# qutech/filter_functions

Hardware: AMD Instinct MI355X
Metric: filter-function elements/sec (n_seg*n_omega*n_nops*d^2) at d=4 (higher is better)
Workload: dtype f64

## Files before the change

### filter_functions_amd/csrc/ctrl_pq.hip

```cpp
#include <algorithm>
#include <cstdlib>

#include "ffk_internal.h"
#include "ffk_mfma_util.h"

namespace ffk {
namespace {

constexpr int kPqProducers = 4;
constexpr int kPqSets = 2;
constexpr int kPqConsumers = 16/kPqSets;
constexpr int kPqRing = 8;
#ifndef FFK_PC_SPIN_LIMIT
#define FFK_PC_SPIN_LIMIT (1 << 21)
#endif
constexpr int kPqSpinLimit = FFK_PC_SPIN_LIMIT;

__device__ __forceinline__ void pq_report_fault(int* fault, int code) {
    if (fault != nullptr && (threadIdx.x & 63) == 0)
        __hip_atomic_store(fault, code, __ATOMIC_RELAXED, __HIP_MEMORY_SCOPE_SYSTEM);
}

typedef double double2_t __attribute__((ext_vector_type(2)));
typedef double double4_t __attribute__((ext_vector_type(4)));
typedef double double8_t __attribute__((ext_vector_type(8)));
typedef int int4_t __attribute__((ext_vector_type(4)));
typedef __attribute__((address_space(3))) int lds_int_t;

template <int NC>
struct PqConsumer;
#include "ctrl_pq_consumer.inc"

constexpr int kPqQ = 0, kPqPsi = 1024, kPqW = 1152;
constexpr int kPqRow = seg_stride(4);
__host__ __device__ constexpr int pq_tile_doubles(int nc) { return kPqW + nc*128 + 32; }
__host__ __device__ constexpr int pq_lds_bytes_for(int nc) {
    return (kPqRing*pq_tile_doubles(nc) + kPqProducers*kPqRow)*8 + 3*kPqRing*4;
}

__device__ __forceinline__ int lds_peek(const int* flag) {
    return __builtin_amdgcn_readfirstlane(*(const volatile lds_int_t*)(flag));
}

template <int NC, bool PRE>
__global__ __launch_bounds__((kPqProducers + kPqConsumers)*64, 3) void ctrl_accumulate_pq_kernel(
    const double* __restrict__ omega, int W, const double* __restrict__ segtab,
    const cplx* __restrict__ ops, int G, int A, int chunk_len, cplx* __restrict__ Ypart,
    const cplx* __restrict__ wfold, int alpha_base, int alpha_end, int* __restrict__ fault_word) {
    constexpr int D = 4, DD = 16, S = kPqRow, TILE = pq_tile_doubles(NC);
    constexpr int TOP = kPqW + NC*128;
    static_assert(PqConsumer<NC>::kTileBytes == TILE*8, "tools/gen_pq_consumer.py and pq_tile_doubles() disagree");
    extern __shared__ __attribute__((aligned(16))) unsigned char lds_raw[];
    double* ring = reinterpret_cast<double*>(lds_raw);
    double* rows = ring + kPqRing*TILE;
    int* ready = reinterpret_cast<int*>(rows + kPqProducers*S);
    int* done = ready + kPqRing;

    const int lane = threadIdx.x & 63;
    const int wave = __builtin_amdgcn_readfirstlane(threadIdx.x >> 6);
    const int alpha0 = alpha_base + blockIdx.y*NC;
    const int n_alpha = min(NC, alpha_end - alpha0);
    const int g0 = blockIdx.z*chunk_len;
    const int g1 = min(G, g0 + chunk_len);
    const int n_it = max(0, g1 - g0);
    int spin_limit = kPqSpinLimit;

    if (threadIdx.x < 3*kPqRing) *(volatile lds_int_t*)(ready + threadIdx.x) = 0;
    __syncthreads();

    if (wave < kPqProducers) {
        __builtin_amdgcn_s_setprio(0);
        const int iw = blockIdx.x*64 + lane;
        double om = omega[iw < W ? iw : W - 1];
        asm volatile("" : "+v"(om));
        const int n_ops = (1 + n_alpha)*DD;
        double* row = rows + wave*S;
        struct Staged {
            cplx o;
            double r0, r1;
        };
        auto request = [&](int it) __attribute__((always_inline)) -> Staged {
            const int g = g0 + it;
            const cplx* src = ops + static_cast<size_t>(g)*(1 + A)*DD;
            const double* st = segtab + static_cast<size_t>(g)*S;
            Staged t;
            if constexpr (PRE) {
                t.o = cplx{0.0, 0.0};
                t.r0 = st[lane];
                t.r1 = st[64 + (lane & (S - 64 - 1))];
            } else {
                t.o = lane < n_ops ? src[lane < DD ? lane : lane + alpha0*DD] : cplx{0.0, 0.0};
                t.r0 = st[lane];
                t.r1 = lane < S - 64 ? st[64 + lane] : 0.0;
            }
            return t;
        };
        auto wait_slot = [&](int slot, int gen) __attribute__((always_inline)) {
            if (gen > 0) {
                int spin = 0;
                for (; spin < spin_limit; ++spin) {
                    if (lds_peek(done + slot) >= gen*kPqConsumers) break;
                    __builtin_amdgcn_s_sleep(2);
                }
                if (spin == spin_limit && spin_limit != 0) {
                    pq_report_fault(fault_word, kFaultPcProducerWait);
                    spin_limit = 0;
                }
                asm volatile("" ::: "memory");
            }
        };
        Staged cur = {};
        if (wave < n_it) cur = request(wave);
        for (int it = wave; it < n_it; it += kPqProducers) {
            const int slot = it & (kPqRing - 1);
            const int gen = it/kPqRing;
            double* buf = ring + slot*TILE;
            row[lane] = cur.r0;
            if (lane < S - 64) row[64 + lane] = cur.r1;
            const cplx o = cur.o;
            if constexpr (PRE) {
                wait_slot(slot, gen);
                const size_t gw = (static_cast<size_t>(g0 + it)*A + alpha0)*64;
#pragma unroll
                for (int a = 0; a < NC; ++a)
                    if (a < n_alpha) lds_dma16(wfold + gw + a*64 + lane, buf + kPqW + a*128);
                if (lane < DD) lds_dma16(ops + static_cast<size_t>(g0 + it)*(1 + A)*DD + lane, buf + TOP);
            }
            if (it + kPqProducers < n_it) cur = request(it + kPqProducers);
            const double* st = row;
            const double2_t sbcb = *reinterpret_cast<const double2_t*>(st + seg_rec(lane >> 2) + 1);
            const double2_t head = *reinterpret_cast<const double2_t*>(st);
            const double sb = sbcb.x, cb = sbcb.y;
            const double dtg = head.x;
            cplx ph;
            sincos_pi<false>(om*head.y, &ph.im, &ph.re);
            double sa, ca;
            sincos_pi<false>(0.5*(om*dtg), &sa, &ca);
            const PhasedFrequency pf = phased_frequency(om, dtg, ph, sa, ca);
            double q[DD];
            auto batch = [&](int e0, int e1) __attribute__((always_inline)) {
                double4_t rec[DD];
#pragma unroll
                for (int e = 0; e < DD; ++e) {
                    if (e < e0 || e >= e1 || (e != 0 && e/D == e%D)) continue;
                    rec[e] = *reinterpret_cast<const double4_t*>(st + seg_rec(e));
                }
                asm volatile("" ::: "memory");
                double xmin = pf.thr;
#pragma unroll
                for (int e = 0; e < DD; ++e) {
                    if (e < e0 || e >= e1 || (e != 0 && e/D == e%D)) continue;
                    const double x = om + rec[e].x;
                    q[e] = fma(pf.sa2, rec[e].z, pf.ca2*rec[e].y)*rcp_fast(x);
                    asm("v_min_f64 %0, |%1|, %0" : "+v"(xmin) : "v"(x));
                }
                if (xmin < pf.thr) {
#pragma unroll
                    for (int e = 0; e < DD; ++e) {
                        if (e < e0 || e >= e1 || (e != 0 && e/D == e%D)) continue;
                        if (fabs(om + rec[e].x) < pf.thr) q[e] = phased_q(pf, rec[e].x, rec[e].y, rec[e].z);
                    }
                }
            };
            batch(0, 8);
            batch(8, 16);
            q[5] = q[0];
            q[10] = q[0];
            q[15] = q[0];
            if constexpr (!PRE) wait_slot(slot, gen);
#pragma unroll
            for (int h = 0; h < 2; ++h)
#pragma unroll
                for (int m = 0; m < D; ++m) {
                    const double2_t v = {q[m*D + 2*h], q[m*D + 2*h + 1]};
                    *reinterpret_cast<double2_t*>(buf + kPqQ + h*512 + lane*8 + (((m ^ (lane >> 2)) & 3) << 1)) = v;
                }
            {
                const double2_t v = {pf.pr, pf.pi};
                *reinterpret_cast<double2_t*>(buf + kPqPsi + lane*2) = v;
            }
            if constexpr (!PRE) {
                const int src_t = lane & (DD - 1);
                const cplx tv = {__shfl(o.re, src_t, 64), __shfl(o.im, src_t, 64)};
                const cplx et = cmul(cplx{cb, sb}, tv);
                const int wslot = ((lane >> 2) & 3)*16 + (lane >> 4)*4 + (lane & 3);
#pragma unroll
                for (int a = 0; a < NC; ++a) {
                    const int src_b = DD + a*DD + (lane >> 2);
                    const cplx bv = {__shfl(o.re, src_b, 64), __shfl(o.im, src_b, 64)};
                    const cplx w = cmul(bv, et);
                    const double2_t v = {w.re, w.im};
                    *reinterpret_cast<double2_t*>(buf + kPqW + a*128 + wslot*2) = v;
                }
            }
            if constexpr (PRE) {
                if (it + kPqProducers < n_it) asm volatile("s_waitcnt vmcnt(2)" ::: "memory");
                else lds_dma_wait();
            } else if (lane < DD) {
                const double2_t v = {o.re, o.im};
                *reinterpret_cast<double2_t*>(buf + TOP + lane*2) = v;
            }
            asm volatile("s_waitcnt lgkmcnt(0)" ::: "memory");
#ifdef FFK_PC_FAULT_INJECT
            if (it < 2*kPqProducers)
#endif
            if (lane == 0) *(volatile lds_int_t*)(ready + slot) = it + 1;
        }
        return;
    }

    const int octant = wave - kPqProducers;
    const int m = lane >> 4, f = (lane >> 2) & 3, j = lane & 3;
    const int mj = m*4 + j;
    const int wf = octant*4*kPqSets + f;
    const int o_w = kPqW + mj*2;
    const int o_p = kPqPsi + wf*2;
    const int o_q0 = kPqQ + wf*8 + ((m ^ ((kPqSets*octant) & 3)) << 1);
    const int o_q1 = (o_q0 ^ 2) + 32;
    double P[6*NC];
#pragma unroll
    for (int k = 0; k < 6*NC; ++k) P[k] = 0.0;
    if (n_it > 0) {
        int spin = 0;
        for (; spin < spin_limit; ++spin) {
            if (lds_peek(ready) >= 1) break;
            __builtin_amdgcn_s_sleep(1);
        }
        if (spin == spin_limit) {
            pq_report_fault(fault_word, kFaultPcConsumerWait);
            spin_limit = 0;
        }
        asm volatile("" ::: "memory");
        const unsigned ring_b = static_cast<unsigned>(reinterpret_cast<uintptr_t>(ring));
        const unsigned flags_b = static_cast<unsigned>(reinterpret_cast<uintptr_t>(ready));
        const int fault_code = PqConsumer<NC>::run(ring_b + o_w*8, ring_b + o_q0*8, ring_b + o_q1*8, ring_b + o_p*8, n_it,
                                                   spin_limit, flags_b, octant, P);
        if (fault_code != 0) pq_report_fault(fault_word, fault_code);
    }
#pragma unroll
    for (int a = 0; a < NC; ++a) {
        const int alpha = alpha0 + a;
        if (alpha >= alpha_end) break;
        cplx* out = Ypart + ((static_cast<size_t>(blockIdx.z)*A + alpha)*DD + mj)*W;
#pragma unroll
        for (int s = 0; s < kPqSets; ++s) {
            const int iw = blockIdx.x*64 + wf + s*4;
            const double p1 = P[3*(kPqSets*a + s)], p2 = P[3*(kPqSets*a + s) + 1], p3 = P[3*(kPqSets*a + s) + 2];
            if (iw < W) out[iw] = cplx{p1 - p2, p3 - (p1 + p2)};
        }
    }
}

template <int NC, bool PRE>
hipError_t launch_pq_as(const double* omega, int W, const double* segtab, const cplx* ops, int G, int A,
                        int chunks, int chunk_len, cplx* Ypart, const cplx* wfold, int alpha_base, int alpha_end,
                        int* fault_word, hipStream_t stream) {
    const int lds = pq_lds_bytes_for(NC);
    auto kern = ctrl_accumulate_pq_kernel<NC, PRE>;
    hipError_t err = hipFuncSetAttribute(reinterpret_cast<const void*>(kern),
                                         hipFuncAttributeMaxDynamicSharedMemorySize, lds);
    if (err != hipSuccess) return err;
    const int n = alpha_end - alpha_base;
    const dim3 grid((W + 63)/64, (n + NC - 1)/NC, chunks);
    hipLaunchKernelGGL(kern, grid, dim3((kPqProducers + kPqConsumers)*64), lds, stream, omega, W, segtab,
                       ops, G, A, chunk_len, Ypart, wfold, alpha_base, alpha_end, fault_word);
    return hipGetLastError();
}

template <int NC>
hipError_t launch_pq(const double* omega, int W, const double* segtab, const cplx* ops, int G, int A,
                     int chunks, int chunk_len, cplx* Ypart, const cplx* wfold, int alpha_base, int alpha_end,
                     int* fault_word, hipStream_t stream) {
    return wfold != nullptr ? launch_pq_as<NC, true>(omega, W, segtab, ops, G, A, chunks, chunk_len, Ypart, wfold,
                                                     alpha_base, alpha_end, fault_word, stream)
                            : launch_pq_as<NC, false>(omega, W, segtab, ops, G, A, chunks, chunk_len, Ypart, nullptr,
                                                      alpha_base, alpha_end, fault_word, stream);
}

}

int pq_accumulate_lds_bytes(int nc) { return pq_lds_bytes_for(nc); }
int pq_accumulate_waves(int) { return kPqProducers + kPqConsumers; }
bool pq_accumulate_supported(int d, int A) { return d == 4 && A >= 1; }

PqGroups pq_accumulate_groups(int A) {
    if (A <= 0) return {0, 0, 0};
    if (A == 1) return {0, 0, 1};
    switch (A % 3) {
        case 0: return {A/3, 0, 0};
        case 1: return {(A - 4)/3, 2, 0};
        default: return {(A - 2)/3, 1, 0};
    }
}

hipError_t launch_accumulate_pq(const double* omega, int W, const double* segtab, const cplx* ops,
                                int G, int d, int A, int chunks, int chunk_len, cplx* Ypart,
                                const cplx* wfold, hipStream_t stream) {
    if (d != 4) return hipErrorInvalidValue;
    int* fault_word = kernel_fault_word();
    const PqGroups g = pq_accumulate_groups(A);
    hipError_t err = hipSuccess;
    int base = 0;
    if (g.n3 > 0) {
        err = launch_pq<3>(omega, W, segtab, ops, G, A, chunks, chunk_len, Ypart, wfold, base, base + 3*g.n3,
                           fault_word, stream);
        base += 3*g.n3;
    }
    if (err == hipSuccess && g.n2 > 0) {
        err = launch_pq<2>(omega, W, segtab, ops, G, A, chunks, chunk_len, Ypart, wfold, base, base + 2*g.n2,
                           fault_word, stream);
        base += 2*g.n2;
    }
    if (err == hipSuccess && g.n1 > 0)
        err = launch_pq<1>(omega, W, segtab, ops, G, A, chunks, chunk_len, Ypart, wfold, base, base + g.n1,
                           fault_word, stream);
    return err;
}

}
```

### filter_functions_amd/csrc/ffk_math.h

```cpp
#pragma once

#include <hip/hip_runtime.h>

#include <cmath>

#define FFK_HD __host__ __device__ __forceinline__

namespace ffk {

struct cplx {
    double re, im;
};

FFK_HD cplx cmul(cplx a, cplx b) {
    return {fma(a.re, b.re, -(a.im*b.im)), fma(a.re, b.im, a.im*b.re)};
}
FFK_HD void cmac(cplx& acc, cplx a, cplx b) {
    acc.re = fma(a.re, b.re, acc.re);
    acc.re = fma(-a.im, b.im, acc.re);
    acc.im = fma(a.re, b.im, acc.im);
    acc.im = fma(a.im, b.re, acc.im);
}
FFK_HD void cmac_conj(cplx& acc, cplx a, cplx b) {
    acc.re = fma(a.re, b.re, acc.re);
    acc.re = fma(a.im, b.im, acc.re);
    acc.im = fma(a.re, b.im, acc.im);
    acc.im = fma(-a.im, b.re, acc.im);
}

template <unsigned long long BITS>
FFK_HD double pinned_bits() {
#if defined(__HIP_DEVICE_COMPILE__)
    unsigned lo, hi;
    asm volatile("v_mov_b32 %0, %1" : "=v"(lo) : "n"(static_cast<unsigned>(BITS & 0xffffffffull)));
    asm volatile("v_mov_b32 %0, %1" : "=v"(hi) : "n"(static_cast<unsigned>(BITS >> 32)));
    return __hiloint2double(static_cast<int>(hi), static_cast<int>(lo));
#else
    return __builtin_bit_cast(double, BITS);
#endif
}
#define FFK_PIN(c) (PIN ? pinned_bits<__builtin_bit_cast(unsigned long long, static_cast<double>(c))>() : (c))

template <bool PIN = false>
FFK_HD void sincos_reduced(double r, double* s, double* c) {
    const double z = r*r;
    double ps = fma(z, FFK_PIN(1.58969099521155010221e-10), FFK_PIN(-2.50507602534068634195e-08));
    ps = fma(z, ps, FFK_PIN(2.75573137070700676789e-06));
    ps = fma(z, ps, FFK_PIN(-1.98412698298579493134e-04));
    ps = fma(z, ps, FFK_PIN(8.33333333332248946124e-03));
    ps = fma(z, ps, FFK_PIN(-1.66666666666666324348e-01));
    *s = fma(r*z, ps, r);
    double pc = fma(z, FFK_PIN(-1.13596475577881948265e-11), FFK_PIN(2.08757232129817482790e-09));
    pc = fma(z, pc, FFK_PIN(-2.75573143513906633035e-07));
    pc = fma(z, pc, FFK_PIN(2.48015872894767294178e-05));
    pc = fma(z, pc, FFK_PIN(-1.38888888888741095749e-03));
    pc = fma(z, pc, FFK_PIN(4.16666666666666019037e-02));
    const double hz = 0.5*z;
    const double w = 1.0 - hz;
    *c = w + (((1.0 - w) - hz) + z*z*pc);
}

template <bool PIN = false>
FFK_HD void sincos_small(double r, double* s, double* c) {
    const double z = r*r;
    double ps = fma(z, FFK_PIN(2.75573137070700676789e-06), FFK_PIN(-1.98412698298579493134e-04));
    ps = fma(z, ps, FFK_PIN(8.33333333332248946124e-03));
    ps = fma(z, ps, FFK_PIN(-1.66666666666666324348e-01));
    *s = fma(r*z, ps, r);
    double pc = fma(z, FFK_PIN(2.48015872894767294178e-05), FFK_PIN(-1.38888888888741095749e-03));
    pc = fma(z, pc, FFK_PIN(4.16666666666666019037e-02));
    const double hz = 0.5*z;
    const double w = 1.0 - hz;
    *c = w + (((1.0 - w) - hz) + z*z*pc);
}

FFK_HD unsigned low_word(double t) {
#if defined(__HIP_DEVICE_COMPILE__)
    return static_cast<unsigned>(__double2loint(t));
#else
    unsigned long long bits;
    __builtin_memcpy(&bits, &t, sizeof bits);
    return static_cast<unsigned>(bits);
#endif
}

template <bool PIN = false>
FFK_HD void sincos_pi(double x, double* s, double* c) {
    const double kMagic = FFK_PIN(6755399441055744.0);
    const double t = fma(x, FFK_PIN(6.36619772367581382433e-01), kMagic);
    const unsigned q = low_word(t);
    const double k = t - kMagic;
    double r = fma(-k, FFK_PIN(1.57079632679489655800e+00), x);
    r = fma(-k, FFK_PIN(6.12323399573676603587e-17), r);
    r = fma(-k, FFK_PIN(-1.49738490485916983294e-33), r);
    double sr, cr;
    sincos_reduced<PIN>(r, &sr, &cr);
    const double s0 = (q & 1u) ? cr : sr;
    const double c0 = (q & 1u) ? sr : cr;
    *s = (q & 2u) ? -s0 : s0;
    *c = ((q + 1u) & 2u) ? -c0 : c0;
}

#undef FFK_PIN

FFK_HD double rcp(double x) {
#if defined(__HIP_DEVICE_COMPILE__)
    double y = __builtin_amdgcn_rcp(x);
    double e = fma(-x, y, 1.0);
    y = fma(y, e, y);
    e = fma(-x, y, 1.0);
    y = fma(y, e, y);
    return y;
#else
    return 1.0/x;
#endif
}

FFK_HD double rcp_fast(double x) {
#if defined(__HIP_DEVICE_COMPILE__)
    double y = __builtin_amdgcn_rcp(x);
    const double e = fma(-x, y, 1.0);
    return fma(y, e, y);
#else
    return 1.0/x;
#endif
}

FFK_HD double rsqrt(double x) {
#if defined(__HIP_DEVICE_COMPILE__)
    double y = __builtin_amdgcn_rsq(x);
    double e = fma(-x*y, y, 1.0);
    y = fma(y, 0.5*e, y);
    e = fma(-x*y, y, 1.0);
    y = fma(y, 0.5*e, y);
    return y;
#else
    return 1.0/sqrt(x);
#endif
}

FFK_HD cplx first_order_integral(double omega, double dE, double dt) {
    const double x = omega + dE;
    const double y = x*dt;
    double s, c;
    sincos_pi(0.5*y, &s, &c);
    const double q = 2.0*s*rcp(x);
    cplx out = {q*c, q*s};
    if (x == 0.0) {
        out.re = dt;
        out.im = 0.0;
    }
    return out;
}

FFK_HD cplx first_order_integral_aa(double omega, double dE, double dt, double sa, double ca,
                                    double sb, double cb) {
    const double x = omega + dE;
    const double h = 0.5*(x*dt);
    double s = fma(sa, cb, ca*sb);
    double c = fma(ca, cb, -(sa*sb));
    if (fabs(h) < 0.03125) sincos_small<true>(h, &s, &c);
    const double q = 2.0*s*rcp_fast(x);
    cplx out = {q*c, q*s};
    if (x == 0.0) {
        out.re = dt;
        out.im = 0.0;
    }
    return out;
}

struct PhasedFrequency {
    double om, dt, thr;
    double pr, pi;
    double sa2, ca2;
};
FFK_HD PhasedFrequency phased_frequency(double om, double dt, cplx ph, double sa, double ca) {
    PhasedFrequency f;
    f.om = om;
    f.dt = dt;
    f.thr = dt > 0.0 ? 0.0625*rcp(dt) : __builtin_huge_val();
    f.pr = fma(ph.re, ca, -(ph.im*sa));
    f.pi = fma(ph.re, sa, ph.im*ca);
    f.sa2 = sa + sa;
    f.ca2 = ca + ca;
    return f;
}
FFK_HD double phased_q(const PhasedFrequency& f, double dE, double sb, double cb) {
    const double x = f.om + dE;
    double q;
    if (fabs(x) < f.thr) {
        double s, c;
        sincos_small<true>(0.5*(x*f.dt), &s, &c);
        q = x == 0.0 ? f.dt : 2.0*s*rcp_fast(x);
    } else {
        q = fma(f.sa2, cb, f.ca2*sb)*rcp_fast(x);
    }
    return q;
}
FFK_HD cplx phased_integral_aa(const PhasedFrequency& f, double dE, double sb, double cb) {
    const double er = fma(f.pr, cb, -(f.pi*sb));
    const double ei = fma(f.pr, sb, f.pi*cb);
    const double q = phased_q(f, dE, sb, cb);
    return {q*er, q*ei};
}

template <bool PIN = false>
FFK_HD cplx cexp(double x) {
    cplx out;
    sincos_pi<PIN>(x, &out.im, &out.re);
    return out;
}

constexpr double kDerivativeIntegralBand = 0.0009765625;
constexpr double kDerivativeIntegralTaylor = 0.001953125;

#define FFK_PINNED(c) pinned_bits<__builtin_bit_cast(unsigned long long, static_cast<double>(c))>()

template <int J>
FFK_HD void derivative_integral_series_step(double X, cplx& S) {
    const double f = X*FFK_PINNED(1.0/(J + 1));
    S = {fma(-f, S.im, FFK_PINNED(1.0/(J + 5))), f*S.re};
    if constexpr (J > 0) derivative_integral_series_step<J - 1>(X, S);
}

FFK_HD double derivative_integral_rcp(double b, double dt) {
    return fabs(b*dt) < kDerivativeIntegralBand ? 0.0 : 1.0/b;
}

FFK_HD cplx derivative_integral_sum(double B, double unit, cplx m1, cplx m2, cplx m3, cplx m4) {
    const double B4 = 0.25*B, B2 = 0.5*B;
    const double B3 = FFK_PINNED(1.0/3.0)*B;
    cplx h = {fma(-B4, m4.im, m3.re), fma(B4, m4.re, m3.im)};
    h = {fma(-B3, h.im, m2.re), fma(B3, h.re, m2.im)};
    h = {fma(-B2, h.im, m1.re), fma(B2, h.re, m1.im)};
    return {unit*h.re, unit*h.im};
}

FFK_HD cplx derivative_integral(double x, double b, double rb, double dt, cplx i1x, cplx i1xb) {
    const cplx df = {i1xb.re - i1x.re, i1xb.im - i1x.im};
    cplx j = {df.im*rb, -df.re*rb};
    const double X = x*dt;
    const double up = rb == 0.0 ? fabs(X) : -1.0, down = rb == 0.0 ? fabs(X) : 1.0;
    if (up >= kDerivativeIntegralTaylor) {
        const cplx ex = {1.0 - x*i1x.im, x*i1x.re};
        const double rx = 1.0/x;
        const cplx m1 = {(dt*ex.im - i1x.im)*rx, -(dt*ex.re - i1x.re)*rx};
        double p = dt*dt;
        const cplx m2 = {(p*ex.im - 2.0*m1.im)*rx, -(p*ex.re - 2.0*m1.re)*rx};
        p *= dt;
        const cplx m3 = {(p*ex.im - 3.0*m2.im)*rx, -(p*ex.re - 3.0*m2.re)*rx};
        p *= dt;
        const cplx m4 = {(p*ex.im - 4.0*m3.im)*rx, -(p*ex.re - 4.0*m3.re)*rx};
        j = derivative_integral_sum(b, 1.0, m1, m2, m3, m4);
    }
    if (down < kDerivativeIntegralTaylor) {
        const cplx ex = {1.0 - x*i1x.im, x*i1x.re};
        cplx m4 = {FFK_PINNED(1.0/10.0), 0.0};
        derivative_integral_series_step<4>(X, m4);
        const double third = FFK_PINNED(1.0/3.0);
        const cplx m3 = {0.25*(ex.re + X*m4.im), 0.25*(ex.im - X*m4.re)};
        const cplx m2 = {(ex.re + X*m3.im)*third, (ex.im - X*m3.re)*third};
        const cplx m1 = {0.5*(ex.re + X*m2.im), 0.5*(ex.im - X*m2.re)};
        j = derivative_integral_sum(b*dt, dt*dt, m1, m2, m3, m4);
    }
    return j;
}

struct SecondOrderMoments {
    cplx m1, m2, m3, m4;
};

FFK_HD SecondOrderMoments second_order_moments(double a, double dt, cplx i1a) {
    const double X = a*dt;
    const cplx ex = {1.0 - a*i1a.im, a*i1a.re};
    SecondOrderMoments m;
    if (fabs(X) >= kDerivativeIntegralTaylor) {
        const double rX = 1.0/X, rdt = 1.0/dt;
        m.m1 = {(ex.im - i1a.im*rdt)*rX, -(ex.re - i1a.re*rdt)*rX};
        m.m2 = {(ex.im - 2.0*m.m1.im)*rX, -(ex.re - 2.0*m.m1.re)*rX};
        m.m3 = {(ex.im - 3.0*m.m2.im)*rX, -(ex.re - 3.0*m.m2.re)*rX};
        m.m4 = {(ex.im - 4.0*m.m3.im)*rX, -(ex.re - 4.0*m.m3.re)*rX};
    } else {
        m.m4 = {0.1, 0.0};
        derivative_integral_series_step<4>(X, m.m4);
        m.m3 = {0.25*(ex.re + X*m.m4.im), 0.25*(ex.im - X*m.m4.re)};
        m.m2 = {(ex.re + X*m.m3.im)*(1.0/3.0), (ex.im - X*m.m3.re)*(1.0/3.0)};
        m.m1 = {0.5*(ex.re + X*m.m2.im), 0.5*(ex.im - X*m.m2.re)};
    }
    return m;
}

FFK_HD cplx second_order_series(double b, double dt, cplx s1, cplx s2, cplx s3, cplx s4) {
    return derivative_integral_sum(b*dt, dt*dt, s1, s2, s3, s4);
}

FFK_HD cplx second_order_integral(double a, double b, double ab, double dt) {
    const cplx i1a = first_order_integral(a, 0.0, dt);
    const double rb = derivative_integral_rcp(b, dt);
    if (rb == 0.0) {
        const SecondOrderMoments m = second_order_moments(a, dt, i1a);
        return second_order_series(b, dt, m.m1, m.m2, m.m3, m.m4);
    }
    const cplx i1ab = first_order_integral(ab, 0.0, dt);
    return {-(i1a.im - i1ab.im)*rb, (i1a.re - i1ab.re)*rb};
}

#undef FFK_PINNED

}
```

### filter_functions_amd/csrc/prep.hip

```cpp
#include "ffk_internal.h"

namespace ffk {
namespace {

template <int D>
__device__ void prologue_segment(const cplx (*V)[D], cplx (*Q)[D], cplx (*T)[D], cplx (*BV)[D],
                                 int g, int lane, const double* __restrict__ eigvals,
                                 const cplx* __restrict__ n_opers,
                                 const double* __restrict__ n_coeffs,
                                 const double* __restrict__ dt, const double* __restrict__ t, int G,
                                 int A, double* __restrict__ segtab, cplx* __restrict__ Tc,
                                 cplx* __restrict__ ops, cplx* __restrict__ n_opers_transformed,
                                 cplx* __restrict__ eigvecs_propagated, bool with_noise_ops = true,
                                 cplx* __restrict__ wfold = nullptr) {
    constexpr int S = seg_stride(D);
    double* st = segtab + static_cast<size_t>(g)*S;
    if (lane == 0) {
        st[0] = dt[g];
        st[1] = t[g];
    }
    cplx eb = {1.0, 0.0};
    for (int e = lane; e < D*D; e += 64) {
        const double dE = eigvals[static_cast<size_t>(g)*D + e / D] - eigvals[static_cast<size_t>(g)*D + e % D];
        double sb, cb;
        sincos_pi(0.5*(dE*dt[g]), &sb, &cb);
        st[seg_rec(e)] = dE;
        st[seg_rec(e) + 1] = sb;
        st[seg_rec(e) + 2] = cb;
        st[seg_rec(e) + 3] = 0.0;
        eb = {cb, sb};
    }
    if (lane < 2) st[2 + lane] = 0.0;
    for (int e = 4 + 4*D*D + lane; e < S; e += 64) st[e] = 0.0;

    for (int e = lane; e < D*D; e += 64) {
        const int m = e / D, j = e % D;
        cplx acc = {0.0, 0.0};
#pragma unroll
        for (int k = 0; k < D; ++k) cmac_conj(acc, V[k][m], Q[k][j]);
        T[m][j] = acc;
        Tc[static_cast<size_t>(g)*D*D + e] = {acc.re, -acc.im};
        ops[static_cast<size_t>(g)*(1 + A)*D*D + e] = acc;
        if (eigvecs_propagated)
            eigvecs_propagated[static_cast<size_t>(g)*D*D + j*D + m] = {acc.re, -acc.im};
    }
    __syncthreads();

    if (!with_noise_ops) return;
    const bool fold = D == 4 && wfold != nullptr;
    if (fold) {
        if (lane < D*D) Q[lane / D][lane % D] = eb;
        __syncthreads();
    }
    for (int a = 0; a < A; ++a) {
        const cplx* B = n_opers + static_cast<size_t>(a)*D*D;
        const double s = n_coeffs ? n_coeffs[static_cast<size_t>(a)*G + g] : 1.0;
        for (int e = lane; e < D*D; e += 64) {
            const int i = e / D, n = e % D;
            cplx acc = {0.0, 0.0};
#pragma unroll
            for (int k = 0; k < D; ++k) cmac(acc, B[i*D + k], V[k][n]);
            BV[i][n] = acc;
        }
        __syncthreads();
        cplx bbar = {0.0, 0.0};
        for (int e = lane; e < D*D; e += 64) {
            const int m = e / D, n = e % D;
            cplx acc = {0.0, 0.0};
#pragma unroll
            for (int k = 0; k < D; ++k) cmac_conj(acc, V[k][m], BV[k][n]);
            acc.re *= s;
            acc.im *= s;
            ops[(static_cast<size_t>(g)*(1 + A) + 1 + a)*D*D + e] = acc;
            if (n_opers_transformed)
                n_opers_transformed[(static_cast<size_t>(a)*G + g)*D*D + e] = acc;
            if (fold) bbar = acc;
        }
        __syncthreads();
        if (fold) {
            if (lane < D*D) BV[lane / D][lane % D] = bbar;
            __syncthreads();
            if constexpr (D == 4) {
                const int m = lane >> 4, n = (lane >> 2) & 3, j = lane & 3;
                const cplx et = cmul(Q[m][n], T[n][j]);
                const cplx w = cmul(BV[m][n], et);
                wfold[(static_cast<size_t>(g)*A + a)*64 + n*16 + m*4 + j] = w;
            }
            __syncthreads();
        }
    }
}

template <int D>
__global__ __launch_bounds__(64) void prologue_kernel(
    const double* __restrict__ eigvals, const cplx* __restrict__ eigvecs,
    const cplx* __restrict__ propagators, const cplx* __restrict__ n_opers,
    const double* __restrict__ n_coeffs, const double* __restrict__ dt,
    const double* __restrict__ t, int G, int A, double* __restrict__ segtab,
    cplx* __restrict__ Tc, cplx* __restrict__ ops, cplx* __restrict__ n_opers_transformed,
    cplx* __restrict__ eigvecs_propagated, bool with_noise_ops, cplx* __restrict__ wfold) {
    __shared__ cplx V[D][D];
    __shared__ cplx Q[D][D];
    __shared__ cplx T[D][D];
    __shared__ cplx BV[D][D];
    const int g = blockIdx.x;
    const int lane = threadIdx.x;
    for (int e = lane; e < D*D; e += 64) {
        V[e / D][e % D] = eigvecs[static_cast<size_t>(g)*D*D + e];
        Q[e / D][e % D] = propagators[static_cast<size_t>(g)*D*D + e];
    }
    __syncthreads();
    prologue_segment<D>(V, Q, T, BV, g, lane, eigvals, n_opers, n_coeffs, dt, t, G, A, segtab, Tc,
                        ops, n_opers_transformed, eigvecs_propagated, with_noise_ops, wfold);
}

template <int D>
__global__ __launch_bounds__(64) void prologue_pulses_kernel(
    const double* __restrict__ eigvals, const cplx* __restrict__ eigvecs,
    const cplx* __restrict__ propagators, const cplx* __restrict__ n_opers,
    const double* __restrict__ n_coeffs, const double* __restrict__ dt,
    const double* __restrict__ t, int G, int A, double* __restrict__ segtab,
    cplx* __restrict__ Tc, cplx* __restrict__ ops, cplx* __restrict__ n_opers_transformed) {
    __shared__ cplx V[D][D];
    __shared__ cplx Q[D][D];
    __shared__ cplx T[D][D];
    __shared__ cplx BV[D][D];
    constexpr size_t DD = D*D;
    const size_t p = blockIdx.y;
    const int g = blockIdx.x;
    const int lane = threadIdx.x;
    const cplx* Vp = eigvecs + p*G*DD;
    const cplx* Qp = propagators + p*(G + 1)*DD;
    for (int e = lane; e < D*D; e += 64) {
        V[e / D][e % D] = Vp[static_cast<size_t>(g)*DD + e];
        Q[e / D][e % D] = Qp[static_cast<size_t>(g)*DD + e];
    }
    __syncthreads();
    prologue_segment<D>(V, Q, T, BV, g, lane, eigvals + p*G*D, n_opers + p*A*DD, n_coeffs + p*A*G, dt + p*G,
                        t + p*(G + 1), G, A, segtab + p*G*seg_stride(D), Tc + p*G*DD, ops + p*G*(1 + A)*DD,
                        n_opers_transformed + p*A*G*DD, nullptr, true, nullptr);
}

template <int D>
__global__ __launch_bounds__(64) void noise_ops_kernel(const cplx* __restrict__ eigvecs,
                                                       const cplx* __restrict__ n_opers,
                                                       const double* __restrict__ n_coeffs, int G,
                                                       int A, cplx* __restrict__ ops,
                                                       cplx* __restrict__ n_opers_transformed) {
    __shared__ cplx V[D][D];
    __shared__ cplx BV[D][D];
    __builtin_amdgcn_s_setprio(3);
    const int g = blockIdx.x, a = blockIdx.y, lane = threadIdx.x;
    for (int e = lane; e < D*D; e += 64) V[e / D][e % D] = eigvecs[static_cast<size_t>(g)*D*D + e];
    __syncthreads();
    const cplx* B = n_opers + static_cast<size_t>(a)*D*D;
    const double s = n_coeffs ? n_coeffs[static_cast<size_t>(a)*G + g] : 1.0;
    for (int e = lane; e < D*D; e += 64) {
        const int i = e / D, n = e % D;
        cplx acc = {0.0, 0.0};
#pragma unroll
        for (int k = 0; k < D; ++k) cmac(acc, B[i*D + k], V[k][n]);
        BV[i][n] = acc;
    }
    __syncthreads();
    for (int e = lane; e < D*D; e += 64) {
        const int m = e / D, n = e % D;
        cplx acc = {0.0, 0.0};
#pragma unroll
        for (int k = 0; k < D; ++k) cmac_conj(acc, V[k][m], BV[k][n]);
        acc.re *= s;
        acc.im *= s;
        ops[(static_cast<size_t>(g)*(1 + A) + 1 + a)*D*D + e] = acc;
        if (n_opers_transformed)
            n_opers_transformed[(static_cast<size_t>(a)*G + g)*D*D + e] = acc;
    }
}

constexpr int kNoiseOpsKernelMinD = 12;
inline bool split_noise_ops(int d, int A) { return d >= kNoiseOpsKernelMinD && A >= 2 && A <= 65535; }

template <int D>
__device__ __forceinline__ void apply_prologue_segment(
    const cplx* __restrict__ Qloc, const cplx* __restrict__ totals, int G, int L,
    cplx* __restrict__ Qout, const double* __restrict__ eigvals, const cplx* __restrict__ eigvecs,
    const cplx* __restrict__ n_opers, const double* __restrict__ n_coeffs,
    const double* __restrict__ dt, const double* __restrict__ t, int A,
    double* __restrict__ segtab, cplx* __restrict__ Tc, cplx* __restrict__ ops,
    bool with_noise_ops, cplx* __restrict__ wfold, const int g) {
    __builtin_amdgcn_s_setprio(3);
    __shared__ cplx E[2][D][D];
    __shared__ cplx M[D][D];
    __shared__ cplx V[D][D];
    __shared__ cplx Q[D][D];
    __shared__ cplx T[D][D];
    __shared__ cplx BV[D][D];
    constexpr int kBatch = 16;
    constexpr bool kTree = D <= 8;
    extern __shared__ __attribute__((aligned(16))) unsigned char tot_raw[];
    cplx (*tot)[D][D] = reinterpret_cast<cplx (*)[D][D]>(tot_raw);
    const int lane = threadIdx.x;
    const int c = g / L;
    for (int e = lane; e < D*D; e += 64) E[0][e / D][e % D] = {(e / D == e % D) ? 1.0 : 0.0, 0.0};
    int b = 0;
    if constexpr (kTree) {
        constexpr int DD = D*D, PER = 64/DD;
        for (int e = lane; e < c*DD; e += 64) (&tot[0][0][0])[e] = totals[e];
        __syncthreads();
        int n = c;
        while (n > 1) {
            const int pairs = n >> 1;
            for (int j0 = 0; j0 < pairs; j0 += PER) {
                const int jj = j0 + lane/DD, e = lane % DD, i = e / D, k = e % D;
                const bool act = lane < PER*DD && jj < pairs;
                cplx acc = {0.0, 0.0};
                if (act) {
#pragma unroll
                    for (int x = 0; x < D; ++x) cmac(acc, tot[2*jj + 1][i][x], tot[2*jj][x][k]);
                }
                __syncthreads();
                if (act) tot[jj][i][k] = acc;
                __syncthreads();
            }
            if (n & 1) {
                const cplx* from = &tot[n - 1][0][0] + (lane < DD ? lane : 0);
                const double carry_re = from->re, carry_im = from->im;
                __syncthreads();
                if (lane < DD) (&tot[pairs][0][0])[lane] = {carry_re, carry_im};
                __syncthreads();
            }
            n = pairs + (n & 1);
        }
        if (c > 0) {
            for (int e = lane; e < DD; e += 64) E[0][e / D][e % D] = tot[0][e / D][e % D];
            __syncthreads();
        }
    } else {
    for (int kb = 0; kb < c; kb += kBatch) {
        const int nb = min(kBatch, c - kb);
        __syncthreads();
        for (int e = lane; e < nb*D*D; e += 64)
            (&tot[0][0][0])[e] = totals[static_cast<size_t>(kb)*D*D + e];
        __syncthreads();
        for (int k = 0; k < nb; ++k) {
            for (int e = lane; e < D*D; e += 64) {
                const int i = e / D, j = e % D;
                cplx acc = {0.0, 0.0};
#pragma unroll
                for (int x = 0; x < D; ++x) cmac(acc, tot[k][i][x], E[b][x][j]);
                E[b ^ 1][i][j] = acc;
            }
            __syncthreads();
            b ^= 1;
        }
    }
    }
    for (int e = lane; e < D*D; e += 64) M[e / D][e % D] = Qloc[static_cast<size_t>(g + 1)*D*D + e];
    if (g == 0)
        for (int e = lane; e < D*D; e += 64) Qout[e] = {(e / D == e % D) ? 1.0 : 0.0, 0.0};
    __syncthreads();
    for (int e = lane; e < D*D; e += 64) {
        const int i = e / D, j = e % D;
        cplx acc = {0.0, 0.0};
#pragma unroll
        for (int x = 0; x < D; ++x) cmac(acc, M[i][x], E[b][x][j]);
        Qout[static_cast<size_t>(g + 1)*D*D + e] = acc;
    }
    if (segtab == nullptr) return;
    __syncthreads();
    if (g % L == 0) {
        for (int e = lane; e < D*D; e += 64) Q[e / D][e % D] = E[b][e / D][e % D];
    } else {
        for (int e = lane; e < D*D; e += 64) M[e / D][e % D] = Qloc[static_cast<size_t>(g)*D*D + e];
        __syncthreads();
        for (int e = lane; e < D*D; e += 64) {
            const int i = e / D, j = e % D;
            cplx acc = {0.0, 0.0};
#pragma unroll
            for (int x = 0; x < D; ++x) cmac(acc, M[i][x], E[b][x][j]);
            Q[i][j] = acc;
        }
    }
    for (int e = lane; e < D*D; e += 64) V[e / D][e % D] = eigvecs[static_cast<size_t>(g)*D*D + e];
    __syncthreads();
    prologue_segment<D>(V, Q, T, BV, g, lane, eigvals, n_opers, n_coeffs, dt, t, G, A, segtab, Tc,
                        ops, nullptr, nullptr, with_noise_ops, wfold);
}

template <int D>
__global__ __launch_bounds__(64) void apply_prologue_kernel(
    const cplx* __restrict__ Qloc, const cplx* __restrict__ totals, int G, int L,
    cplx* __restrict__ Qout, const double* __restrict__ eigvals, const cplx* __restrict__ eigvecs,
    const cplx* __restrict__ n_opers, const double* __restrict__ n_coeffs,
    const double* __restrict__ dt, const double* __restrict__ t, int A,
    double* __restrict__ segtab, cplx* __restrict__ Tc, cplx* __restrict__ ops,
    const cplx* __restrict__ basis, int* __restrict__ nnz, int* __restrict__ rows,
    cplx* __restrict__ vals, bool with_noise_ops, cplx* __restrict__ wfold) {
    if (static_cast<int>(blockIdx.x) >= G) {
        basis_compact_one(basis, D, static_cast<int>(blockIdx.x) - G, threadIdx.x, nnz, rows, vals);
        return;
    }
    apply_prologue_segment<D>(Qloc, totals, G, L, Qout, eigvals, eigvecs, n_opers, n_coeffs, dt, t, A, segtab, Tc,
                              ops, with_noise_ops, wfold, blockIdx.x);
}

template <int D>
__global__ __launch_bounds__(64) void apply_prologue_pulses_kernel(
    const cplx* __restrict__ Qloc, const cplx* __restrict__ totals, int G, int L, int nchunks,
    cplx* __restrict__ Qout, const double* __restrict__ eigvals, const cplx* __restrict__ eigvecs,
    const cplx* __restrict__ n_opers, const double* __restrict__ n_coeffs,
    const double* __restrict__ dt, const double* __restrict__ t, int A,
    double* __restrict__ segtab, cplx* __restrict__ Tc, cplx* __restrict__ ops,
    const cplx* __restrict__ basis, int* __restrict__ nnz, int* __restrict__ rows,
    cplx* __restrict__ vals, cplx* __restrict__ wfold) {
    const size_t p = blockIdx.y;
    if (static_cast<int>(blockIdx.x) >= G) {
        if (p == 0) basis_compact_one(basis, D, static_cast<int>(blockIdx.x) - G, threadIdx.x, nnz, rows, vals);
        return;
    }
    constexpr size_t DD = D*D;
    apply_prologue_segment<D>(Qloc + p*(G + 1)*DD, totals + p*nchunks*DD, G, L, Qout + p*(G + 1)*DD,
                              eigvals + p*G*D, eigvecs + p*G*DD, n_opers + p*A*DD, n_coeffs + p*A*G, dt + p*G,
                              t + p*(G + 1), A, segtab + p*G*seg_stride(D), Tc + p*G*DD, ops + p*G*(1 + A)*DD,
                              true, wfold ? wfold + p*G*A*64 : nullptr, blockIdx.x);
}

template <int D>
__global__ __launch_bounds__(64) void basis_transformed_kernel(const cplx* __restrict__ Tc,
                                                               const cplx* __restrict__ basis,
                                                               int N, cplx* __restrict__ out) {
    __shared__ cplx T[D][D];
    __shared__ cplx C[D][D];
    __shared__ cplx TC[D][D];
    const int g = blockIdx.x, k = blockIdx.y, lane = threadIdx.x;
    for (int e = lane; e < D*D; e += 64) {
        const cplx v = Tc[static_cast<size_t>(g)*D*D + e];
        T[e / D][e % D] = {v.re, -v.im};
        C[e / D][e % D] = basis[static_cast<size_t>(k)*D*D + e];
    }
    __syncthreads();
    for (int e = lane; e < D*D; e += 64) {
        const int i = e / D, j = e % D;
        cplx acc = {0.0, 0.0};
#pragma unroll
        for (int a = 0; a < D; ++a) cmac(acc, T[i][a], C[a][j]);
        TC[i][j] = acc;
    }
    __syncthreads();
    for (int e = lane; e < D*D; e += 64) {
        const int i = e / D, j = e % D;
        cplx acc = {0.0, 0.0};
#pragma unroll
        for (int a = 0; a < D; ++a) {
            const cplx tj = T[j][a];
            cmac_conj(acc, tj, TC[i][a]);
        }
        out[(static_cast<size_t>(g)*N + k)*D*D + e] = acc;
    }
}

__global__ void phase_integral_kernel(const double* __restrict__ omega, int W,
                                      const double* __restrict__ segtab, int d, int S,
                                      cplx* __restrict__ phase_factors,
                                      cplx* __restrict__ integral) {
    const int g = blockIdx.x;
    const int w = blockIdx.y*blockDim.x + threadIdx.x;
    if (w >= W) return;
    const double* st = segtab + static_cast<size_t>(g)*S;
    const double om = omega[w];
    if (phase_factors) phase_factors[static_cast<size_t>(g)*W + w] = cexp(om*st[1]);
    if (integral) {
        cplx* out = integral + (static_cast<size_t>(g)*W + w)*d*d;
        for (int e = 0; e < d*d; ++e) out[e] = first_order_integral(om, st[seg_rec(e)], st[0]);
    }
}

}

__global__ __launch_bounds__(64) void fold_w8_kernel(const double* __restrict__ segtab, const cplx* __restrict__ ops,
                                                     int A, cplx* __restrict__ wfold) {
    constexpr int D = 8, DD = 64, S = seg_stride(8);
    const int g = blockIdx.x, a = blockIdx.y, lane = threadIdx.x;
    const cplx* src = ops + static_cast<size_t>(g)*(1 + A)*DD;
    const double* r = segtab + static_cast<size_t>(g)*S + seg_rec(lane);
    const cplx x = src[static_cast<size_t>(1 + a)*DD + lane];
    const double sb = r[1], cb = r[2];
    const int m = lane >> 3, n = lane & 7;
    const int base = ((m >> 2)*2 + (n >> 2))*2*64 + 4*(n & 3) + 16*(m & 3);
    const cplx bt = cmul(x, cplx{cb, sb});
    cplx* out = wfold + (static_cast<size_t>(g)*A + a)*512;
#pragma unroll
    for (int i = 0; i < D; ++i) {
        const cplx t = src[m*D + i];
        out[base + (i >> 2)*64 + (i & 3)] = cmul(bt, cplx{t.re, -t.im});
    }
}

hipError_t launch_fold_w8(const double* segtab, const cplx* ops, int G, int A, cplx* wfold, hipStream_t stream) {
    hipLaunchKernelGGL(fold_w8_kernel, dim3(G, A), dim3(64), 0, stream, segtab, ops, A, wfold);
    return hipGetLastError();
}

hipError_t launch_prologue(const double* eigvals, const cplx* eigvecs, const cplx* propagators,
                           const cplx* n_opers, const double* n_coeffs, const double* dt,
                           const double* t, int G, int d, int A, double* segtab, cplx* Tc,
                           cplx* ops, cplx* n_opers_transformed, cplx* eigvecs_propagated,
                           hipStream_t stream, cplx* wfold) {
    if (generic_dimension(d))
        return launch_prologue_generic(eigvals, eigvecs, propagators, n_opers, n_coeffs, dt, t, G, d, A, segtab,
                                       Tc, ops, n_opers_transformed, eigvecs_propagated, stream);
    switch (d) {
#define FFK_CASE(D)                                                                             \
    case D:                                                                                     \
        hipLaunchKernelGGL(prologue_kernel<D>, dim3(G), dim3(64), 0, stream, eigvals, eigvecs,  \
                           propagators, n_opers, n_coeffs, dt, t, G, A, segtab, Tc, ops,        \
                           n_opers_transformed, eigvecs_propagated, !split_noise_ops(D, A),     \
                           D == 4 ? wfold : nullptr);                                           \
        if (split_noise_ops(D, A))                                                              \
            hipLaunchKernelGGL(noise_ops_kernel<D>, dim3(G, A), dim3(64), 0, stream, eigvecs,   \
                               n_opers, n_coeffs, G, A, ops, n_opers_transformed);              \
        break;
        FFK_CASE(2) FFK_CASE(3) FFK_CASE(4) FFK_CASE(5) FFK_CASE(6) FFK_CASE(7) FFK_CASE(8)
        FFK_CASE(9) FFK_CASE(10) FFK_CASE(11) FFK_CASE(12) FFK_CASE(13) FFK_CASE(14)
        FFK_CASE(15) FFK_CASE(16)
#undef FFK_CASE
        default:
            return hipErrorInvalidValue;
    }
    if (d == 8 && wfold != nullptr) return launch_fold_w8(segtab, ops, G, A, wfold, stream);
    return hipGetLastError();
}

hipError_t launch_prologue_pulses(const double* eigvals, const cplx* eigvecs, const cplx* propagators,
                                  const cplx* n_opers, const double* n_coeffs, const double* dt, const double* t,
                                  int G, int P, int d, int A, double* segtab, cplx* Tc, cplx* ops,
                                  cplx* n_opers_transformed, hipStream_t stream) {
    if (P < 1 || P > 65535 || !n_opers_transformed || !n_coeffs) return hipErrorInvalidValue;
    switch (d) {
#define FFK_CASE(D)                                                                             \
    case D:                                                                                     \
        hipLaunchKernelGGL(prologue_pulses_kernel<D>, dim3(G, P), dim3(64), 0, stream, eigvals, \
                           eigvecs, propagators, n_opers, n_coeffs, dt, t, G, A, segtab, Tc,    \
                           ops, n_opers_transformed);                                           \
        break;
        FFK_CASE(2) FFK_CASE(3) FFK_CASE(4) FFK_CASE(5) FFK_CASE(6) FFK_CASE(7) FFK_CASE(8)
#undef FFK_CASE
        default:
            return hipErrorInvalidValue;
    }
    return hipGetLastError();
}

hipError_t launch_apply_prologue_compact(const cplx* Qloc, const cplx* totals, int G, int d, cplx* Q,
                                         const double* eigvals, const cplx* eigvecs,
                                         const cplx* n_opers, const double* n_coeffs,
                                         const double* dt, const double* t, int A, double* segtab,
                                         cplx* Tc, cplx* ops, const cplx* basis, int N, void* ews,
                                         hipStream_t stream, cplx* wfold) {
    const int L = front_chunk(d);
    int* nnz = nullptr;
    int* rows = nullptr;
    cplx* vals = nullptr;
    int extra = 0;
    if (basis) {
        expand_workspace_slices(ews, N, d, &nnz, &rows, &vals);
        extra = N;
    }
    switch (d) {
#define FFK_CASE(D)                                                                              \
    case D:                                                                                      \
        if (D > 8) {    \
            hipError_t e = hipFuncSetAttribute(reinterpret_cast<const void*>(apply_prologue_kernel<D>), \
                                               hipFuncAttributeMaxDynamicSharedMemorySize,       \
                                               static_cast<int>(sizeof(cplx)*D*D*16));           \
            if (e != hipSuccess) return e;                                                       \
        }                                                                                        \
        hipLaunchKernelGGL(apply_prologue_kernel<D>, dim3(G + extra), dim3(64),                  \
                           sizeof(cplx)*D*D*(D <= 8 ? (G + L - 1)/L : 16), stream, Qloc,         \
                           totals, G, L, Q, eigvals, eigvecs, n_opers, n_coeffs, dt, t, A,       \
                           segtab, Tc, ops, basis, nnz, rows, vals, !split_noise_ops(D, A),      \
                           D == 4 ? wfold : nullptr);                                            \
        if (split_noise_ops(D, A))                                                               \
            hipLaunchKernelGGL(noise_ops_kernel<D>, dim3(G, A), dim3(64), 0, stream, eigvecs,    \
                               n_opers, n_coeffs, G, A, ops, nullptr);                           \
        break;
        FFK_CASE(2) FFK_CASE(3) FFK_CASE(4) FFK_CASE(5) FFK_CASE(6) FFK_CASE(7) FFK_CASE(8)
        FFK_CASE(9) FFK_CASE(10) FFK_CASE(11) FFK_CASE(12) FFK_CASE(13) FFK_CASE(14)
        FFK_CASE(15) FFK_CASE(16)
#undef FFK_CASE
        default:
            return hipErrorInvalidValue;
    }
    if (d == 8 && wfold != nullptr) return launch_fold_w8(segtab, ops, G, A, wfold, stream);
    return hipGetLastError();
}

hipError_t launch_apply_prologue_compact_pulses(const cplx* Qloc, const cplx* totals, int G, int P, int d,
                                                cplx* Q, const double* eigvals, const cplx* eigvecs,
                                                const cplx* n_opers, const double* n_coeffs, const double* dt,
                                                const double* t, int A, double* segtab, cplx* Tc, cplx* ops,
                                                const cplx* basis, int N, void* ews, hipStream_t stream,
                                                cplx* wfold) {
    const int L = front_chunk(d);
    const int nchunks = (G + L - 1)/L;
    if (P < 1 || P > 65535 || !basis) return hipErrorInvalidValue;
    int* nnz = nullptr;
    int* rows = nullptr;
    cplx* vals = nullptr;
    expand_workspace_slices(ews, N, d, &nnz, &rows, &vals);
    switch (d) {
#define FFK_CASE(D)                                                                              \
    case D:                                                                                      \
        if (D > 8) {                                                                             \
            hipError_t e = hipFuncSetAttribute(reinterpret_cast<const void*>(apply_prologue_pulses_kernel<D>), \
                                               hipFuncAttributeMaxDynamicSharedMemorySize,       \
                                               static_cast<int>(sizeof(cplx)*D*D*16));           \
            if (e != hipSuccess) return e;                                                       \
        }                                                                                        \
        hipLaunchKernelGGL(apply_prologue_pulses_kernel<D>, dim3(G + N, P), dim3(64),            \
                           sizeof(cplx)*D*D*(D <= 8 ? nchunks : 16), stream, Qloc, totals, G, L, \
                           nchunks, Q, eigvals, eigvecs, n_opers, n_coeffs, dt, t, A, segtab, Tc, \
                           ops, basis, nnz, rows, vals, D == 4 ? wfold : nullptr);               \
        break;
        FFK_CASE(2) FFK_CASE(3) FFK_CASE(4) FFK_CASE(5) FFK_CASE(6) FFK_CASE(7) FFK_CASE(8)
        FFK_CASE(9) FFK_CASE(10) FFK_CASE(11) FFK_CASE(12) FFK_CASE(13) FFK_CASE(14)
        FFK_CASE(15) FFK_CASE(16)
#undef FFK_CASE
        default:
            return hipErrorInvalidValue;
    }
    if (d == 8 && wfold != nullptr) return launch_fold_w8(segtab, ops, P*G, A, wfold, stream);
    return hipGetLastError();
}

hipError_t launch_apply_prologue(const cplx* Qloc, const cplx* totals, int G, int d, cplx* Q,
                                 const double* eigvals, const cplx* eigvecs, const cplx* n_opers,
                                 const double* n_coeffs, const double* dt, const double* t, int A,
                                 double* segtab, cplx* Tc, cplx* ops, hipStream_t stream) {
    return launch_apply_prologue_compact(Qloc, totals, G, d, Q, eigvals, eigvecs, n_opers, n_coeffs,
                                         dt, t, A, segtab, Tc, ops, nullptr, 0, nullptr, stream);
}

hipError_t launch_basis_transformed(const cplx* Tc, const cplx* basis, int G, int N, int d,
                                    cplx* out, hipStream_t stream) {
    if (N > 65535) return hipErrorInvalidValue;
    switch (d) {
#define FFK_CASE(D)                                                                            \
    case D:                                                                                    \
        hipLaunchKernelGGL(basis_transformed_kernel<D>, dim3(G, N), dim3(64), 0, stream, Tc,   \
                           basis, N, out);                                                     \
        break;
        FFK_CASE(2) FFK_CASE(3) FFK_CASE(4) FFK_CASE(5) FFK_CASE(6) FFK_CASE(7) FFK_CASE(8)
        FFK_CASE(9) FFK_CASE(10) FFK_CASE(11) FFK_CASE(12) FFK_CASE(13) FFK_CASE(14)
        FFK_CASE(15) FFK_CASE(16)
#undef FFK_CASE
        default:
            return hipErrorInvalidValue;
    }
    return hipGetLastError();
}

hipError_t launch_phase_and_integral(const double* omega, int W, const double* segtab, int G,
                                     int d, cplx* phase_factors, cplx* integral,
                                     hipStream_t stream) {
    if (!phase_factors && !integral) return hipSuccess;
    const int block = 128;
    if ((W + block - 1)/block > 65535) return hipErrorInvalidValue;
    hipLaunchKernelGGL(phase_integral_kernel, dim3(G, (W + block - 1)/block), dim3(block), 0,
                       stream, omega, W, segtab, d, seg_stride(d), phase_factors, integral);
    return hipGetLastError();
}

}
```

Measured before the change: 911.1 billion.

## Exploit antisymmetric eigenvalue pairs to share reciprocals in producer q computation

Producer waves now compute q for each (i,j)/(j,i) pair of the d=4 eigenvalue difference table together. The mirror entry has negated dE and sb, so one reciprocal of (om+dE)(om-dE) serves both, and the pair loads half as many records. The threshold 1/dt is precomputed into the segment table during prep, and the diagonal entry uses a hoisted 1/om. Pairs whose product leaves a safe range fall back to the exact per-entry path, which adds branching and slightly different rounding.

```diff
diff --git a/filter_functions_amd/csrc/ctrl_pq.hip b/filter_functions_amd/csrc/ctrl_pq.hip
--- a/filter_functions_amd/csrc/ctrl_pq.hip
+++ b/filter_functions_amd/csrc/ctrl_pq.hip
@@ -15,6 +15,11 @@
 #define FFK_PC_SPIN_LIMIT (1 << 21)
 #endif
 constexpr int kPqSpinLimit = FFK_PC_SPIN_LIMIT;
+constexpr int kPqPairs = 6;
+__host__ __device__ constexpr int pq_pair_entry(int k) { return k < 3 ? 1 + k : (k < 5 ? 3 + k : 11); }
+__host__ __device__ constexpr int pq_mirror_entry(int k) { return (pq_pair_entry(k) & 3)*4 + (pq_pair_entry(k) >> 2); }
+static_assert(pq_pair_entry(3) == 6 && pq_pair_entry(4) == 7 && pq_mirror_entry(4) == 13 && pq_mirror_entry(5) == 14,
+              "pairs of d = 4");
 
 __device__ __forceinline__ void pq_report_fault(int* fault, int code) {
     if (fault != nullptr && (threadIdx.x & 63) == 0)
@@ -72,7 +77,6 @@
         __builtin_amdgcn_s_setprio(0);
         const int iw = blockIdx.x*64 + lane;
         double om = omega[iw < W ? iw : W - 1];
-        asm volatile("" : "+v"(om));
         const int n_ops = (1 + n_alpha)*DD;
         double* row = rows + wave*S;
         struct Staged {
@@ -111,6 +115,8 @@
         };
         Staged cur = {};
         if (wave < n_it) cur = request(wave);
+        asm volatile("" : "+v"(om));
+        const double inv_om = rcp_fast(om);
         for (int it = wave; it < n_it; it += kPqProducers) {
             const int slot = it & (kPqRing - 1);
             const int gen = it/kPqRing;
@@ -130,40 +136,61 @@
             const double* st = row;
             const double2_t sbcb = *reinterpret_cast<const double2_t*>(st + seg_rec(lane >> 2) + 1);
             const double2_t head = *reinterpret_cast<const double2_t*>(st);
+            const double2_t band = *reinterpret_cast<const double2_t*>(st + 2);
             const double sb = sbcb.x, cb = sbcb.y;
             const double dtg = head.x;
             cplx ph;
             sincos_pi<false>(om*head.y, &ph.im, &ph.re);
             double sa, ca;
             sincos_pi<false>(0.5*(om*dtg), &sa, &ca);
-            const PhasedFrequency pf = phased_frequency(om, dtg, ph, sa, ca);
+            const PhasedFrequency pf = phased_frequency(om, dtg, band.x, ph, sa, ca);
             double q[DD];
-            auto batch = [&](int e0, int e1) __attribute__((always_inline)) {
-                double4_t rec[DD];
-#pragma unroll
-                for (int e = 0; e < DD; ++e) {
-                    if (e < e0 || e >= e1 || (e != 0 && e/D == e%D)) continue;
-                    rec[e] = *reinterpret_cast<const double4_t*>(st + seg_rec(e));
+            auto batch = [&](int k0, int k1) __attribute__((always_inline)) {
+                double2_t ds[kPqPairs + 1];
+                double c[kPqPairs + 1];
+#pragma unroll
+                for (int k = 0; k <= kPqPairs; ++k) {
+                    if (k < kPqPairs ? (k < k0 || k >= k1) : k0 != 0) continue;
+                    const double* r = st + seg_rec(k < kPqPairs ? pq_pair_entry(k) : 0);
+                    ds[k] = *reinterpret_cast<const double2_t*>(r);
+                    c[k] = r[2];
                 }
                 asm volatile("" ::: "memory");
-                double xmin = pf.thr;
-#pragma unroll
-                for (int e = 0; e < DD; ++e) {
-                    if (e < e0 || e >= e1 || (e != 0 && e/D == e%D)) continue;
-                    const double x = om + rec[e].x;
-                    q[e] = fma(pf.sa2, rec[e].z, pf.ca2*rec[e].y)*rcp_fast(x);
+                double xmin = pf.thr, pmax = 0.0;
+                if (k0 == 0) {
+                    const double x = om + ds[kPqPairs].x;
+                    q[0] = fma(pf.sa2, c[kPqPairs], pf.ca2*ds[kPqPairs].y)*inv_om;
                     asm("v_min_f64 %0, |%1|, %0" : "+v"(xmin) : "v"(x));
                 }
-                if (xmin < pf.thr) {
-#pragma unroll
-                    for (int e = 0; e < DD; ++e) {
-                        if (e < e0 || e >= e1 || (e != 0 && e/D == e%D)) continue;
-                        if (fabs(om + rec[e].x) < pf.thr) q[e] = phased_q(pf, rec[e].x, rec[e].y, rec[e].z);
+#pragma unroll
+                for (int k = 0; k < kPqPairs; ++k) {
+                    if (k < k0 || k >= k1) continue;
+                    const PhasedPair p = phased_q_pair(pf, ds[k].x, ds[k].y, c[k]);
+                    q[pq_pair_entry(k)] = p.qp;
+                    q[pq_mirror_entry(k)] = p.qm;
+                    asm("v_min_f64 %0, |%1|, %0" : "+v"(xmin) : "v"(p.xp));
+                    asm("v_min_f64 %0, |%1|, %0" : "+v"(xmin) : "v"(p.xm));
+                    asm("v_max_f64 %0, |%1|, %0" : "+v"(pmax) : "v"(p.prod));
+                }
+                const bool wide = !(pmax < kPhasedPairRange);
+                if (xmin < pf.thr || wide) {
+                    if (k0 == 0 && fabs(om + ds[kPqPairs].x) < pf.thr)
+                        q[0] = phased_q(pf, ds[kPqPairs].x, ds[kPqPairs].y, c[kPqPairs]);
+#pragma unroll
+                    for (int k = 0; k < kPqPairs; ++k) {
+                        if (k < k0 || k >= k1) continue;
+                        const double xp = om + ds[k].x, xm = om - ds[k].x;
+                        double xnear;
+                        asm("v_min_f64 %0, |%1|, |%2|" : "=v"(xnear) : "v"(xp), "v"(xm));
+                        if (xnear < pf.thr || wide) {
+                            q[pq_pair_entry(k)] = phased_q(pf, ds[k].x, ds[k].y, c[k]);
+                            q[pq_mirror_entry(k)] = phased_q(pf, -ds[k].x, -ds[k].y, c[k]);
+                        }
                     }
                 }
             };
-            batch(0, 8);
-            batch(8, 16);
+            batch(0, 3);
+            batch(3, kPqPairs);
             q[5] = q[0];
             q[10] = q[0];
             q[15] = q[0];
diff --git a/filter_functions_amd/csrc/ffk_math.h b/filter_functions_amd/csrc/ffk_math.h
--- a/filter_functions_amd/csrc/ffk_math.h
+++ b/filter_functions_amd/csrc/ffk_math.h
@@ -174,16 +174,22 @@
     double pr, pi;
     double sa2, ca2;
 };
-FFK_HD PhasedFrequency phased_frequency(double om, double dt, cplx ph, double sa, double ca) {
+FFK_HD double phased_threshold(double dt) {
+    return dt > 0.0 ? 0.0625*rcp(dt) : __builtin_huge_val();
+}
+FFK_HD PhasedFrequency phased_frequency(double om, double dt, double thr, cplx ph, double sa, double ca) {
     PhasedFrequency f;
     f.om = om;
     f.dt = dt;
-    f.thr = dt > 0.0 ? 0.0625*rcp(dt) : __builtin_huge_val();
+    f.thr = thr;
     f.pr = fma(ph.re, ca, -(ph.im*sa));
     f.pi = fma(ph.re, sa, ph.im*ca);
     f.sa2 = sa + sa;
     f.ca2 = ca + ca;
     return f;
+}
+FFK_HD PhasedFrequency phased_frequency(double om, double dt, cplx ph, double sa, double ca) {
+    return phased_frequency(om, dt, phased_threshold(dt), ph, sa, ca);
 }
 FFK_HD double phased_q(const PhasedFrequency& f, double dE, double sb, double cb) {
     const double x = f.om + dE;
@@ -196,6 +202,24 @@
         q = fma(f.sa2, cb, f.ca2*sb)*rcp_fast(x);
     }
     return q;
+}
+struct PhasedPair {
+    double qp, qm;
+    double xp, xm, prod;
+};
+constexpr double kPhasedPairRange = 0x1p+960;
+FFK_HD PhasedPair phased_q_pair(const PhasedFrequency& f, double dE, double sb, double cb) {
+    PhasedPair p;
+    p.xp = f.om + dE;
+    p.xm = f.om - dE;
+    const double u = f.ca2*sb;
+    const double sp = fma(f.sa2, cb, u);
+    const double sm = fma(f.sa2, cb, -u);
+    p.prod = p.xp*p.xm;
+    const double r = rcp_fast(p.prod);
+    p.qp = (sp*p.xm)*r;
+    p.qm = (sm*p.xp)*r;
+    return p;
 }
 FFK_HD cplx phased_integral_aa(const PhasedFrequency& f, double dE, double sb, double cb) {
     const double er = fma(f.pr, cb, -(f.pi*sb));
diff --git a/filter_functions_amd/csrc/prep.hip b/filter_functions_amd/csrc/prep.hip
--- a/filter_functions_amd/csrc/prep.hip
+++ b/filter_functions_amd/csrc/prep.hip
@@ -30,7 +30,7 @@
         st[seg_rec(e) + 3] = 0.0;
         eb = {cb, sb};
     }
-    if (lane < 2) st[2 + lane] = 0.0;
+    if (lane < 2) st[2 + lane] = lane == 0 ? phased_threshold(dt[g]) : 0.0;
     for (int e = 4 + 4*D*D + lane; e < S; e += 64) st[e] = 0.0;
 
     for (int e = lane; e < D*D; e += 64) {
```

Result: no change. 917.7 billion, median of 6 (+0.7%).
